# facebookresearch/hyperreel

Measured on NVIDIA H100. Metric: Mrays/s at 65k-ray x 32-sample batch, higher is better.
Workload: dtype f32 (sample net bf16x3 split on wgmma, fp32 accumulate)

## Files before the change

### hyperreel_b200/csrc/hr_api.cu

```cuda
#include <cuda_runtime.h>

#include <cmath>
#include <cstdarg>
#include <cstdio>
#include <cstring>
#include <limits>
#include <new>
#include <string>
#include <vector>

#include "hr_common.cuh"
#include "hr_encode.cuh"
#include "hr_geom.cuh"
#include "hr_mlp.cuh"
#include "hyperreel_b200.h"

namespace hr {
cudaError_t launch_render(const hr_config& cfg, const Derived& dv, const RenderTabs& tabs, const float* rays,
                          const float* heads, const RgbDst& rgb, long long n, const ExtraOut* so, int num_sms,
                          cudaStream_t stream, unsigned char* rgb8);
cudaError_t launch_render_bwd(const hr_config& cfg, const Derived& dv, const RenderTabs& tabs, const GradTabs& gt, const float* rays,
                              const float* heads, const float* d_rgb, float* d_heads, long long n, int clamp_output, int white_bg,
                              int num_sms, cudaStream_t stream);
cudaError_t launch_generate_rays(const hr_camera& cam, int c_in, long long first, long long n, float* out, cudaStream_t st);
// ... 6 lines not shown
static thread_local std::string g_err;

int hr_fail(const char* fmt, ...) {
  char buf[1024];
  va_list ap;
  va_start(ap, fmt);
  vsnprintf(buf, sizeof(buf), fmt, ap);
  va_end(ap);
  g_err = buf;
  return 1;
}

struct DeviceGuard {
  int prev = -1;
  bool switched = false;
  explicit DeviceGuard(int dev) {
    if (cudaGetDevice(&prev) == cudaSuccess && prev != dev) switched = (cudaSetDevice(dev) == cudaSuccess);
  }
  ~DeviceGuard() {
    if (switched) cudaSetDevice(prev);
  }
};

#define CK(expr)                                                                                                        \
  do {                                                                                                                  \
    cudaError_t _e = (expr);                                                                                            \
    if (_e != cudaSuccess) return hr_fail("%s failed: %s (%s:%d)", #expr, cudaGetErrorString(_e), __FILE__, __LINE__); \
  } while (0)

#include "hr_handle.h"

namespace {

__global__ void pack_channel_last(const float* __restrict__ src, float* __restrict__ dst, int C, int H, int W) {
  long long total = (long long)C * H * W;
  for (long long i = blockIdx.x * (long long)blockDim.x + threadIdx.x; i < total; i += (long long)gridDim.x * blockDim.x) {
    int c = (int)(i % C);
    long long hw = i / C;
    dst[i] = src[(long long)c * H * W + hw];
  }
}

__global__ void pack_time_lines(const float* __restrict__ src, float* __restrict__ dst, int C, int K, int L, float inv_fac,
                                float time_scale, float time_offset) {
  long long total = (long long)K * L * C;
  for (long long i = blockIdx.x * (long long)blockDim.x + threadIdx.x; i < total; i += (long long)gridDim.x * blockDim.x) {
    int c = (int)(i % C);
    int l = (int)((i / C) % L);
    int k = (int)(i / ((long long)C * L));
    float ft;
    int it = hr::keyframe_blend(k, K, inv_fac, time_scale, time_offset, ft);
    float a = src[((long long)c * K + it) * L + l];
    float b = src[((long long)c * K + it + 1) * L + l];
    dst[i] = __fmul_rn(1.0f - ft, a) + __fmul_rn(ft, b);
  }
}

__global__ void pack_simt_layer(const float* __restrict__ Wsrc, const float* __restrict__ bsrc, float* __restrict__ Wt,
                                float* __restrict__ bias, int Kp, int Np, int out_ch, int in_ch_src, int in_enc,
                                int in_pad, int has_input, int has_hidden, int width, int perm_S, int perm_stride) {
  long long total = (long long)Kp * Np;
  for (long long i = blockIdx.x * (long long)blockDim.x + threadIdx.x; i < total + Np; i += (long long)gridDim.x * blockDim.x) {
    if (i >= total) {
      int n = (int)(i - total);
      int ns = n;
      if (perm_S > 0 && n < out_ch) ns = (n % perm_S) * perm_stride + (n / perm_S);
      bias[n] = (n < out_ch) ? bsrc[ns] : 0.0f;
      continue;
    }
    int n = (int)(i % Np);
    int k = (int)(i / Np);
    float v = 0.0f;
    if (n < out_ch) {
      int ns = n;
      if (perm_S > 0) ns = (n % perm_S) * perm_stride + (n / perm_S);
      int ks = -1;
      if (has_input) {
        if (k < in_pad) ks = (k < in_enc) ? k : -1;
        else if (has_hidden) ks = in_enc + (k - in_pad);
      } else {
        ks = k;
      }
      if (ks >= 0 && ks < in_ch_src && (has_input || k < width)) v = Wsrc[(long long)ns * in_ch_src + ks];
    }
    Wt[i] = v;
  }
}
// ... 303 lines not shown
    float *Wt = nullptr, *bias = nullptr;
    if ((r = dev_alloc(h, (void**)&Wt, (size_t)Kp * Np * sizeof(float)))) break;
    if ((r = dev_alloc(h, (void**)&bias, (size_t)Np * sizeof(float)))) break;
    pack_simt_layer<<<grid_for((long long)Kp * Np + Np), 256, 0, st>>>(
        w_dev[l], b_dev[l], Wt, bias, Kp, Np, out_ch, in_src, nc.mlp_in, in_pad, (first || skip) ? 1 : 0, skip ? 1 : 0, W,
        last ? nc.n_samples : 0, nc.head_stride);
    simt.Wt[l] = Wt;
    simt.bias[l] = bias;
    simt.Kp[l] = Kp;
    simt.Np[l] = Np;
  }
  if (!r && nc.mlp_mode == HR_MLP_BF16X3_TC) {
    r = hr::pack_mlp_tc2(net, w_dev, b_dev, st);
    if (!r) net.tc_ready = true;
  }
  return r;
}

int hr_upload(hr_handle* h, const hr_params* p, void* stream) {
  if (!h || !p) return hr_fail("hr_upload: null argument");
  DeviceGuard guard(h->device);
  drop_host_graph(h);
  cudaStream_t st = (cudaStream_t)stream;
  const hr_config& c = h->cfg;
  h->slot_cursor = 0;
  h->uploaded = false;
  h->net.tc_ready = h->pre.tc_ready = false;
  std::vector<void*> temps;
  int rc = 0;

  rc = pack_net(h, h->net, p->mlp_weight, p->mlp_bias, p->on_device, st, temps);
  if (!rc && c.cascade) rc = pack_net(h, h->pre, p->pre_mlp_weight, p->pre_mlp_bias, p->on_device, st, temps);

  auto pack_tab = [&](const float* src, int C, int H, int Wd, const float** out) -> int {
    *out = nullptr;
    if (C == 0) return 0;
    if (!src) return hr_fail("hr_upload: table with C=%d missing", C);
    const float* d = nullptr;
    if (stage_in(src, (size_t)C * H * Wd, p->on_device, st, temps, &d)) return 1;
    float* dst = nullptr;
    if (dev_alloc(h, (void**)&dst, (size_t)C * H * Wd * sizeof(float))) return 1;
    pack_channel_last<<<grid_for((long long)C * H * Wd), 256, 0, st>>>(d, dst, C, H, Wd);
    *out = dst;
    return 0;
  };
  int n_app_total = 0;
  for (int i = 0; i < 3 && !rc; ++i) {
    const int C = c.n_sigma[i];
    n_app_total += c.n_app[i];
    const int H2 = c.dynamic ? c.num_keyframes : 1;
    hr::PlaneTab& ts = h->tabs.sig[i];
    hr::PlaneTab& ta = h->tabs.app[i];
    ts.C = C; ta.C = c.n_app[i];
    ts.H = ta.H = p->plane_h[i];
    ts.W = ta.W = p->plane_w[i];
    ts.H2 = ta.H2 = H2;
    ts.L = ta.L = p->second_len[i];
    if (C > 0 && (ts.H < 2 || ts.W < 2 || ts.L < 2)) { rc = hr_fail("hr_upload: plane %d too small (%dx%d, L=%d)", i, ts.H, ts.W, ts.L); break; }
    if ((rc = pack_tab(p->sigma_plane[i], C, ts.H, ts.W, &ts.space))) break;
    if ((rc = pack_tab(p->app_plane[i], C, ts.H, ts.W, &ta.space))) break;
    if (!c.dynamic) {
      if ((rc = pack_tab(p->sigma_second[i], C, H2, ts.L, &ts.second))) break;
      if ((rc = pack_tab(p->app_second[i], C, H2, ts.L, &ta.second))) break;
    } else if (C > 0) {
      if (H2 < 2) { rc = hr_fail("hr_upload: the keyframe (time) planes need at least 2 keyframes"); break; }
      for (int f = 0; f < 2 && !rc; ++f) {
        const float* srcp = f ? p->app_second[i] : p->sigma_second[i];
        if (!srcp) { rc = hr_fail("hr_upload: time plane %d missing", i); break; }
        const float* d = nullptr;
        if ((rc = stage_in(srcp, (size_t)C * H2 * ts.L, p->on_device, st, temps, &d))) break;
        float* dst = nullptr;
        if ((rc = dev_alloc(h, (void**)&dst, (size_t)C * H2 * ts.L * sizeof(float)))) break;
        pack_time_lines<<<grid_for((long long)C * H2 * ts.L), 256, 0, st>>>(d, dst, C, H2, ts.L, h->dv.time_inv_fac,
                                                                            h->dv.time_scale, h->dv.time_offset);
        (f ? ta.second : ts.second) = dst;
      }
      if (rc) break;
    }
  }
  if (!rc) {
    const int rx = p->plane_w[0], ry = p->plane_h[0], rz = p->second_len[0];
    h->dv.res[0] = rx; h->dv.res[1] = ry; h->dv.res[2] = rz;
    h->dv.kt = c.dynamic ? c.num_keyframes : 1;
    if (c.dynamic && c.num_keyframes < 2) rc = hr_fail("hr_upload: the keyframe (time) planes need at least 2 keyframes");
    if (c.n_sigma[1] > 0 && (p->plane_w[1] != rx || p->plane_h[1] != rz || p->second_len[1] != ry))
      rc = hr_fail("hr_upload: table group 1 is inconsistent with grid %dx%dx%d", rx, ry, rz);
    if (!rc && c.n_sigma[2] > 0 && (p->plane_w[2] != ry || p->plane_h[2] != rz || p->second_len[2] != rx))
      rc = hr_fail("hr_upload: table group 2 is inconsistent with grid %dx%dx%d", rx, ry, rz);
  }
  if (!rc) {
    if (!p->basis_mat) rc = hr_fail("hr_upload: basis_mat missing");
    else {
      const float* d = nullptr;
      size_t cnt = (size_t)c.app_dim * n_app_total;
      rc = stage_in(p->basis_mat, cnt, p->on_device, st, temps, &d);
      if (!rc) {
        float* dst = nullptr;
        rc = dev_alloc(h, (void**)&dst, cnt * sizeof(float));
        if (!rc) {
          cudaError_t e = cudaMemcpyAsync(dst, d, cnt * sizeof(float), cudaMemcpyDeviceToDevice, st);
          if (e != cudaSuccess) rc = hr_fail("basis copy failed: %s", cudaGetErrorString(e));
          h->tabs.basis = dst;
          h->tabs.n_app_total = n_app_total;
        }
      }
    }
  }
  if (!rc) {
    h->tabs.color_embedding = nullptr;
    if (c.n_color_views > 0) {
      if (!p->color_embedding) rc = hr_fail("hr_upload: color_embedding missing (n_color_views = %d)", c.n_color_views);
// ... 1053 lines not shown
```

### hyperreel_b200/csrc/hr_common.cuh

```cuda
#pragma once
#include <cuda_runtime.h>
#include <stdint.h>
#include "hyperreel_b200.h"

namespace hr {

struct PlaneTab {
  const float* space;
  const float* second;
  int H, W;
  int H2, L;
  int C;
};

struct RenderTabs {
  PlaneTab sig[3];
  PlaneTab app[3];
  const float* basis;
  int n_app_total;
  const float* color_embedding;
};

struct GradTabs {
  float* sig_space[3];
  float* sig_second[3];
  float* app_space[3];
  float* app_second[3];
  float* basis;
  float* color_embedding;
};

struct Derived {
  float time_fac;
  float time_inv_fac;
  float time_scale;
  float time_offset;
  float kf_max;
  float inv_end_dist;
  float dist_scale_fac;
  float inv_end_rad;
  float rad_scale_fac;
  int res[3];
  int kt;
};

struct RgbDst {
// ... 49 lines not shown
```

### hyperreel_b200/csrc/hr_render_bwd_kernel.cuh

```cuda
#pragma once
#include "hr_common.cuh"
#include "hr_geom.cuh"

namespace hr {

static constexpr int kBwdWarps = 4;

__device__ __forceinline__ float act_grad(const hr_act& a, float x) {
  const float v = __fadd_rn(__fmul_rn(x, a.inner_fac), a.shift);
  float g = 1.0f;
  if (a.kind == HR_ACT_SIGMOID) {
    const float s = 1.0f / (1.0f + expf(-v));
    g = s * (1.0f - s);
  } else if (a.kind == HR_ACT_TANH) {
    const float t = tanhf(v);
    g = 1.0f - t * t;
  }
  return g * a.inner_fac * a.outer_fac;
}

__device__ __forceinline__ float act_grad_eased(const hr_act& a, float x) {
  const float g = act_grad(a, x);
  return a.eased ? g * a.ease_mul : g;
}
// ... 81 lines not shown
    g[2] = (hz - hu * uz) / nn * cfg.plane_normal_scale;
    g[3] = cfg.z_scale * dpd_dpre / ddn;
  }
}

__device__ __forceinline__ void contract_point_vjp(const hr_config& cfg, const Derived& dv, float px, float py, float pz,
                                                   float& vx, float& vy, float& vz) {
  const float sr = cfg.contract_start_radius;
  const float x = px / sr, y = py / sr, z = pz / sr;
  const float r = sqrtf(x * x + y * y + z * z);
  if (r < 1.0f) {
    vx /= sr; vy /= sr; vz /= sr;
    return;
  }
  const float k0 = 2.0f + dv.inv_end_rad * dv.rad_scale_fac;
  const float g = k0 / r - dv.rad_scale_fac / (r * r);
  const float gp = -k0 / (r * r) + 2.0f * dv.rad_scale_fac / (r * r * r);
  const float xv = x * vx + y * vy + z * vz;
  const float s = gp / r * xv;
  vx = (g * vx + s * x) / sr;
  vy = (g * vy + s * y) / sr;
  vz = (g * vz + s * z) / sr;
}

__device__ __forceinline__ void red_add4(float* p, float a, float b, float c, float d) {
  asm volatile("red.global.add.v4.f32 [%0], {%1, %2, %3, %4};" ::"l"(p), "f"(a), "f"(b), "f"(c), "f"(d) : "memory");
}

struct Quad {
  float A[4], dAa[4], dAb[4];
  float B[4], dBc[4];
};

template <int C>
__device__ __forceinline__ void quad_fetch(Quad& q, const PlaneTab& T, int ia, int ib, int ic, int krow, int ch0, float fa, float fb,
                                           float fc) {
  const float* s0 = T.space + ((long long)(ib * T.W + ia) * C + ch0);
  const float4 v00 = ldg4(s0), v10 = ldg4(s0 + C), v01 = ldg4(s0 + (long long)T.W * C), v11 = ldg4(s0 + (long long)T.W * C + C);
  const float* e0 = T.second + ((long long)(krow * T.L + ic) * C + ch0);
  const float4 l0 = ldg4(e0), l1 = ldg4(e0 + C);
  const float a00[4] = {v00.x, v00.y, v00.z, v00.w}, a10[4] = {v10.x, v10.y, v10.z, v10.w};
  const float a01[4] = {v01.x, v01.y, v01.z, v01.w}, a11[4] = {v11.x, v11.y, v11.z, v11.w};
  const float b0[4] = {l0.x, l0.y, l0.z, l0.w}, b1[4] = {l1.x, l1.y, l1.z, l1.w};
#pragma unroll
  for (int c = 0; c < 4; ++c) {
    const float top = a00[c] + fa * (a10[c] - a00[c]);
    const float bot = a01[c] + fa * (a11[c] - a01[c]);
    q.A[c] = top + fb * (bot - top);
    q.dAa[c] = (1.0f - fb) * (a10[c] - a00[c]) + fb * (a11[c] - a01[c]);
    q.dAb[c] = bot - top;
    q.B[c] = b0[c] + fc * (b1[c] - b0[c]);
    q.dBc[c] = b1[c] - b0[c];
  }
}

template <int C>
__device__ __forceinline__ void quad_scatter(const Quad& q, const float (&g)[4], float* gspace, float* gsecond, const PlaneTab& T,
                                             int ia, int ib, int ic, int krow, int ch0, float fa, float fb, float fc, float& dfa,
                                             float& dfb, float& dfc) {
  float gA[4], gB[4];
#pragma unroll
  for (int c = 0; c < 4; ++c) {
    gA[c] = g[c] * q.B[c];
    gB[c] = g[c] * q.A[c];
    dfa += gA[c] * q.dAa[c];
    dfb += gA[c] * q.dAb[c];
    dfc += gB[c] * q.dBc[c];
  }
  float* s0 = gspace + ((long long)(ib * T.W + ia) * C + ch0);
  const float w00 = (1.0f - fa) * (1.0f - fb), w10 = fa * (1.0f - fb), w01 = (1.0f - fa) * fb, w11 = fa * fb;
  red_add4(s0, w00 * gA[0], w00 * gA[1], w00 * gA[2], w00 * gA[3]);
  red_add4(s0 + C, w10 * gA[0], w10 * gA[1], w10 * gA[2], w10 * gA[3]);
  red_add4(s0 + (long long)T.W * C, w01 * gA[0], w01 * gA[1], w01 * gA[2], w01 * gA[3]);
  red_add4(s0 + (long long)T.W * C + C, w11 * gA[0], w11 * gA[1], w11 * gA[2], w11 * gA[3]);
  float* e0 = gsecond + ((long long)(krow * T.L + ic) * C + ch0);
  const float u0 = 1.0f - fc, u1 = fc;
  red_add4(e0, u0 * gB[0], u0 * gB[1], u0 * gB[2], u0 * gB[3]);
  red_add4(e0 + C, u1 * gB[0], u1 * gB[1], u1 * gB[2], u1 * gB[3]);
}

struct BwdOpts {
  int clamp_output;
  int white_bg;
};

template <int SPL, bool DYN, int C0, int C1, int C2, int SHADE, bool RARE, bool EASE>
__global__ void __launch_bounds__(kBwdWarps * 32)
render_bwd_kernel(const __grid_constant__ hr_config cfg, const __grid_constant__ Derived dv,
                  const __grid_constant__ RenderTabs tabs, const __grid_constant__ GradTabs gt, const float* __restrict__ rays,
                  const float* __restrict__ heads, const float* __restrict__ d_rgb, float* __restrict__ d_heads,
                  long long n_rays, BwdOpts opt) {
  constexpr int NT = C0 + C1 + C2;
  constexpr int ROWS = (SHADE == HR_SHADE_SH) ? 9 : 1;
  constexpr int NB = 3 * ROWS * NT;
  extern __shared__ float smem[];
  float* s_basis = smem;
  float* s_gbasis = smem + NB;
  float* s_warp = smem + 2 * NB;
  constexpr int WARP_FLOATS = 3 * NT + 12 + 64;
  float* s_gemb = s_warp + kBwdWarps * WARP_FLOATS;
  const int n_emb = RARE ? 12 * cfg.n_color_views : 0;
  for (int i = threadIdx.x; i < NB; i += blockDim.x) { s_basis[i] = tabs.basis[i]; s_gbasis[i] = 0.0f; }
  if constexpr (RARE) {
    for (int i = threadIdx.x; i < n_emb; i += blockDim.x) s_gemb[i] = 0.0f;
  }
  __syncthreads();

  const int lane = threadIdx.x & 31, wib = threadIdx.x >> 5;
  float* Gs = s_warp + wib * WARP_FLOATS;
  float* Ys = Gs + 3 * NT;
  float* perm = Ys + 12;
  const int S = cfg.n_samples;
  const int out_stride = cfg.mlp_out;
  const long long warp0 = (long long)blockIdx.x * kBwdWarps + wib;
  const long long nwarps = (long long)gridDim.x * kBwdWarps;
  const float inv_x = __fdiv_rn(2.0f, __fsub_rn(cfg.aabb[3], cfg.aabb[0]));
  const float inv_y = __fdiv_rn(2.0f, __fsub_rn(cfg.aabb[4], cfg.aabb[1]));
  const float inv_z = __fdiv_rn(2.0f, __fsub_rn(cfg.aabb[5], cfg.aabb[2]));
  const float tsx = inv_x * 0.5f * (float)(dv.res[0] - 1), tsy = inv_y * 0.5f * (float)(dv.res[1] - 1),
              tsz = inv_z * 0.5f * (float)(dv.res[2] - 1);

  for (long long ray = warp0; ray < n_rays; ray += nwarps) {
    const float* r = rays + ray * cfg.c_in;
    const float* hrow = heads + ray * (long long)out_stride;
    float* grow = d_heads + ray * (long long)out_stride;
    const float ox = __ldg(r + 0), oy = __ldg(r + 1), oz = __ldg(r + 2);
    const float dx = __ldg(r + 3), dy = __ldg(r + 4), dz = __ldg(r + 5);
// ... 144 lines not shown
      dist[j] = t;
      const bool inside = !((cfg.aabb[0] > px) || (px > cfg.aabb[3]) || (cfg.aabb[1] > py) || (py > cfg.aabb[4]) ||
                            (cfg.aabb[2] > pz) || (pz > cfg.aabb[5]));
      valid[j] = act && inside && (t > 0.0f);
      const float ux = __fsub_rn(__fmul_rn(__fsub_rn(px, cfg.aabb[0]), inv_x), 1.0f);
      const float uy = __fsub_rn(__fmul_rn(__fsub_rn(py, cfg.aabb[1]), inv_y), 1.0f);
      const float uz = __fsub_rn(__fmul_rn(__fsub_rn(pz, cfg.aabb[2]), inv_z), 1.0f);
      const float tx = __fmul_rn(__fmul_rn(__fadd_rn(ux, 1.0f), 0.5f), (float)(dv.res[0] - 1));
      const float ty = __fmul_rn(__fmul_rn(__fadd_rn(uy, 1.0f), 0.5f), (float)(dv.res[1] - 1));
      const float tz = __fmul_rn(__fmul_rn(__fadd_rn(uz, 1.0f), 0.5f), (float)(dv.res[2] - 1));
      ix[j] = max(0, min((int)floorf(tx), dv.res[0] - 2));
      iy[j] = max(0, min((int)floorf(ty), dv.res[1] - 2));
      iz[j] = max(0, min((int)floorf(tz), dv.res[2] - 2));
      fx[j] = tx - (float)ix[j];
      fy[j] = ty - (float)iy[j];
      fz[j] = tz - (float)iz[j];
      if (!valid[j]) { ix[j] = 0; iy[j] = 0; iz[j] = 0; }
    }

    float feat[SPL], pre[SPL][3];
#pragma unroll
    for (int j = 0; j < SPL; ++j) {
      float sf = 0.0f, pr[3] = {0.0f, 0.0f, 0.0f};
      if (valid[j]) {
        int n0 = 0;
#pragma unroll
        for (int grp = 0; grp < 3; ++grp) {
          const int C = (grp == 0) ? C0 : ((grp == 1) ? C1 : C2);
          if (C == 0) continue;
          const int ia = (grp == 2) ? iy[j] : ix[j], ib = (grp == 0) ? iy[j] : iz[j], ic = (grp == 0) ? iz[j] : ((grp == 1) ? iy[j] : ix[j]);
          const float fa = (grp == 2) ? fy[j] : fx[j], fb = (grp == 0) ? fy[j] : fz[j], fc = (grp == 0) ? fz[j] : ((grp == 1) ? fy[j] : fx[j]);
          for (int ch0 = 0; ch0 < C; ch0 += 4) {
            Quad q;
            if (C == 8) quad_fetch<8>(q, tabs.sig[grp], ia, ib, ic, krow, ch0, fa, fb, fc);
            else quad_fetch<4>(q, tabs.sig[grp], ia, ib, ic, krow, ch0, fa, fb, fc);
#pragma unroll
            for (int c = 0; c < 4; ++c) sf = fmaf(q.A[c], q.B[c], sf);
            if (C == 8) quad_fetch<8>(q, tabs.app[grp], ia, ib, ic, krow, ch0, fa, fb, fc);
            else quad_fetch<4>(q, tabs.app[grp], ia, ib, ic, krow, ch0, fa, fb, fc);
#pragma unroll
            for (int c = 0; c < 4; ++c) {
              const float f = q.A[c] * q.B[c];
              const int n = n0 + ch0 + c;
              pr[0] = fmaf(Gs[n], f, pr[0]);
              pr[1] = fmaf(Gs[NT + n], f, pr[1]);
              pr[2] = fmaf(Gs[2 * NT + n], f, pr[2]);
            }
          }
          n0 += C;
        }
      }
      feat[j] = sf;
      pre[j][0] = pr[0]; pre[j][1] = pr[1]; pre[j][2] = pr[2];
    }

    float sigma[SPL], delta[SPL], ex[SPL], Tt[SPL], wgt[SPL], a1s[SPL];
    float cs[SPL][3], csh[SPL][3], rgbv[SPL][3];
    float carryT = 1.0f, accw = 0.0f, accC[3] = {0.f, 0.f, 0.f};
#pragma unroll
    for (int j = 0; j < SPL; ++j) {
      const int s = lane + 32 * j;
      const float* hp = hrow + ((s < S) ? s : 0);
      float sgm = feature2density(cfg, feat[j]);
      if (!valid[j]) sgm = 0.0f;
      sigma[j] = sgm;
      const SampleAlpha sa = sample_alpha<SPL>(dist, j, sigma[j], cfg.distance_scale, lane, S);
      delta[j] = sa.delta;
      ex[j] = sa.ex;
      a1s[j] = sa.a1;
      Tt[j] = transmittance<32>(sa.a1, lane, carryT);
      wgt[j] = sa.alpha * Tt[j];
      accw += wgt[j];
// ... 121 lines not shown
#pragma unroll
    for (int j = 0; j < SPL; ++j) {
      float prev = __shfl_up_sync(kFull, g_delta[j], 1);
      if (lane == 0) prev = (j > 0) ? __shfl_sync(kFull, g_delta[(j > 0) ? j - 1 : 0], 31) : 0.0f;
      else if (j > 0) (void)__shfl_sync(kFull, g_delta[j - 1], 31);
      g_dist[j] = prev - g_delta[j];
    }

    float g_head_cs[SPL][3], g_head_csh[SPL][3];
    float g_p[SPL][3];
#pragma unroll
    for (int j = 0; j < SPL; ++j) {
      const int s = lane + 32 * j;
      float gt3[3] = {0.0f, 0.0f, 0.0f};
      float g_feat = 0.0f;
      if (valid[j]) {
        if (cfg.fea2dense == HR_DENSE_RELU) g_feat = (feat[j] > 0.0f) ? g_sigma[j] : 0.0f;
        else if (cfg.fea2dense == HR_DENSE_RELU_ABS) g_feat = (feat[j] > 0.0f) ? g_sigma[j] : ((feat[j] < 0.0f) ? -g_sigma[j] : 0.0f);
        else { const float xs = feat[j] + cfg.density_shift; g_feat = g_sigma[j] / (1.0f + expf(-xs)); }
      }
      const bool any_app = (g_pre[j][0] != 0.0f) || (g_pre[j][1] != 0.0f) || (g_pre[j][2] != 0.0f);
      int n0 = 0;
#pragma unroll
      for (int grp = 0; grp < 3; ++grp) {
        const int C = (grp == 0) ? C0 : ((grp == 1) ? C1 : C2);
        if (C == 0) continue;
        const int ia = (grp == 2) ? iy[j] : ix[j], ib = (grp == 0) ? iy[j] : iz[j], ic = (grp == 0) ? iz[j] : ((grp == 1) ? iy[j] : ix[j]);
        const float fa = (grp == 2) ? fy[j] : fx[j], fb = (grp == 0) ? fy[j] : fz[j], fc = (grp == 0) ? fz[j] : ((grp == 1) ? fy[j] : fx[j]);
        float dfa = 0.0f, dfb = 0.0f, dfc = 0.0f;
        for (int ch0 = 0; ch0 < C; ch0 += 4) {
          Quad q;
          if (valid[j] && g_feat != 0.0f) {
            const float g4[4] = {g_feat, g_feat, g_feat, g_feat};
            if (C == 8) { quad_fetch<8>(q, tabs.sig[grp], ia, ib, ic, krow, ch0, fa, fb, fc); quad_scatter<8>(q, g4, gt.sig_space[grp], gt.sig_second[grp], tabs.sig[grp], ia, ib, ic, krow, ch0, fa, fb, fc, dfa, dfb, dfc); }
            else { quad_fetch<4>(q, tabs.sig[grp], ia, ib, ic, krow, ch0, fa, fb, fc); quad_scatter<4>(q, g4, gt.sig_space[grp], gt.sig_second[grp], tabs.sig[grp], ia, ib, ic, krow, ch0, fa, fb, fc, dfa, dfb, dfc); }
          }
          float m[3][4];
#pragma unroll
          for (int c = 0; c < 3; ++c)
#pragma unroll
            for (int k = 0; k < 4; ++k) m[c][k] = 0.0f;
          if (valid[j] && any_app) {
            if (C == 8) quad_fetch<8>(q, tabs.app[grp], ia, ib, ic, krow, ch0, fa, fb, fc);
            else quad_fetch<4>(q, tabs.app[grp], ia, ib, ic, krow, ch0, fa, fb, fc);
            float g4[4];
#pragma unroll
            for (int k = 0; k < 4; ++k) {
              const int n = n0 + ch0 + k;
              g4[k] = g_pre[j][0] * Gs[n] + g_pre[j][1] * Gs[NT + n] + g_pre[j][2] * Gs[2 * NT + n];
              const float f = q.A[k] * q.B[k];
              m[0][k] = g_pre[j][0] * f; m[1][k] = g_pre[j][1] * f; m[2][k] = g_pre[j][2] * f;
            }
            if (C == 8) quad_scatter<8>(q, g4, gt.app_space[grp], gt.app_second[grp], tabs.app[grp], ia, ib, ic, krow, ch0, fa, fb, fc, dfa, dfb, dfc);
            else quad_scatter<4>(q, g4, gt.app_space[grp], gt.app_second[grp], tabs.app[grp], ia, ib, ic, krow, ch0, fa, fb, fc, dfa, dfb, dfc);
          }
#pragma unroll
          for (int c = 0; c < 3; ++c)
#pragma unroll
            for (int k = 0; k < 4; ++k) {
              float v = m[c][k];
#pragma unroll
              for (int d = 1; d < 32; d <<= 1) v += __shfl_xor_sync(kFull, v, d);
              m[c][k] = v;
            }
          if constexpr (SHADE == HR_SHADE_SH) {
            for (int e = lane; e < 108; e += 32) {
              const int c = e / 36, rem = e % 36, kk = rem / 4, k = rem % 4;
              float v = (c == 0) ? m[0][0] : 0.0f;
#pragma unroll
              for (int cc = 0; cc < 3; ++cc)
#pragma unroll
                for (int k2 = 0; k2 < 4; ++k2)
                  if (cc == c && k2 == k) v = m[cc][k2];
              atomicAdd(&s_gbasis[(c * 9 + kk) * NT + n0 + ch0 + k], Ys[kk] * v);
            }
          } else {
            if (lane < 12) {
// ... 204 lines not shown
```

### hyperreel_b200/csrc/hr_render_kernel.cuh

```cuda
#pragma once
#include "hr_common.cuh"
#include "hr_geom.cuh"

namespace hr {

static constexpr int kWarpsPerCta = 8;
static constexpr int kMinCtasPerSm = 3;

template <int C, bool ROWS2>
struct Taps {
  float4 a, b;
};

template <int C, bool ROWS2>
__device__ __forceinline__ void fetch(Taps<C, ROWS2>& t, const float* __restrict__ tab, int off, int rs) {
  t.a = ldg4(tab + off);
  if constexpr (C == 8 && ROWS2) t.b = ldg4(tab + off + rs);
}

template <int C>
__device__ __forceinline__ void plane_share(const Taps<C, true>& t, float fa, float fb, int xt, int alt, float (&out)[4]) {
  const float wa = xt ? fa : 1.0f - fa;
  if constexpr (C == 8) {
    const float w0 = wa * (1.0f - fb), w1 = wa * fb;
    out[0] = fmaf(w1, t.b.x, w0 * t.a.x);
    out[1] = fmaf(w1, t.b.y, w0 * t.a.y);
    out[2] = fmaf(w1, t.b.z, w0 * t.a.z);
    out[3] = fmaf(w1, t.b.w, w0 * t.a.w);
  } else {
    const float w = wa * (alt ? fb : 1.0f - fb);
    out[0] = w * t.a.x; out[1] = w * t.a.y; out[2] = w * t.a.z; out[3] = w * t.a.w;
  }
}

template <int C>
__device__ __forceinline__ void line_full(const Taps<C, false>& t, float fc, int xt, float (&out)[4]) {
  const float wc = xt ? fc : 1.0f - fc;
  out[0] = wc * t.a.x; out[1] = wc * t.a.y; out[2] = wc * t.a.z; out[3] = wc * t.a.w;
#pragma unroll
  for (int c = 0; c < 4; ++c) out[c] += __shfl_xor_sync(kFull, out[c], 2);
}

template <int C, bool DYN>
struct GroupTaps {
  Taps<C, true> sp;
  Taps<C, false> se;
};

template <int C, bool DYN>
__device__ __forceinline__ void group_fetch(GroupTaps<C, DYN>& g, const PlaneTab& T, int ia, int ib, int ic, int krow, int xt,
                                            int alt, bool ok) {
  int so, eo;
  if constexpr (C == 8) {
    so = ((ib * T.W + ia + xt) << 3) + (alt << 2);
    eo = ((krow * T.L + ic + xt) << 3) + (alt << 2);
  } else {
    so = ((ib + alt) * T.W + ia + xt) << 2;
    eo = (krow * T.L + ic + xt) << 2;
  }
  so = ok ? so : 0;
  eo = ok ? eo : 0;
  fetch<C, true>(g.sp, T.space, so, T.W * C);
  fetch<C, false>(g.se, T.second, eo, 0);
}

template <int C, bool DYN>
__device__ __forceinline__ float group_sigma(const GroupTaps<C, DYN>& g, float fa, float fb, float fc, int xt, int alt) {
  float P[4], L[4];
  plane_share<C>(g.sp, fa, fb, xt, alt, P);
  line_full<C>(g.se, fc, xt, L);
  float s = (P[0] * L[0] + P[1] * L[1]) + (P[2] * L[2] + P[3] * L[3]);
  s += __shfl_xor_sync(kFull, s, 2);
  s += __shfl_xor_sync(kFull, s, 1);
  return s;
}

template <int C, bool DYN>
__device__ __forceinline__ void group_app(const GroupTaps<C, DYN>& g, float fa, float fb, float fc, int xt, int alt,
                                          float (&prod)[4]) {
  float P[4], L[4];
  plane_share<C>(g.sp, fa, fb, xt, alt, P);
  line_full<C>(g.se, fc, xt, L);
#pragma unroll
  for (int c = 0; c < 4; ++c) {
    P[c] += __shfl_xor_sync(kFull, P[c], 2);
    if constexpr (C == 4) P[c] += __shfl_xor_sync(kFull, P[c], 1);
    prod[c] = P[c] * L[c];
  }
}

template <int C, bool DYN>
__device__ __forceinline__ void group_accumulate(const GroupTaps<C, DYN>& sg, const GroupTaps<C, DYN>& ag, float fa, float fb,
                                                 float fc, int xt, int alt, const float* __restrict__ G0,
                                                 const float* __restrict__ G1, const float* __restrict__ G2, float (&v)[4]) {
  float P[4], L[4];
  plane_share<C>(sg.sp, fa, fb, xt, alt, P);
  line_full<C>(sg.se, fc, xt, L);
  v[3] += (P[0] * L[0] + P[1] * L[1]) + (P[2] * L[2] + P[3] * L[3]);
  plane_share<C>(ag.sp, fa, fb, xt, alt, P);
  line_full<C>(ag.se, fc, xt, L);
#pragma unroll
  for (int c = 0; c < 4; ++c) {
    const float t = P[c] * L[c];
    v[0] = fmaf(G0[c], t, v[0]);
    v[1] = fmaf(G1[c], t, v[1]);
    v[2] = fmaf(G2[c], t, v[2]);
  }
}

__device__ __forceinline__ float quad_transpose_reduce(const float (&v)[4], int xt, int alt) {
  const float x = __shfl_xor_sync(kFull, xt ? v[0] : v[2], 2);
  const float y = __shfl_xor_sync(kFull, xt ? v[1] : v[3], 2);
  const float k0 = (xt ? v[2] : v[0]) + x;
  const float k1 = (xt ? v[3] : v[1]) + y;
  const float z = __shfl_xor_sync(kFull, alt ? k0 : k1, 1);
  return (alt ? k1 : k0) + z;
}

template <int SPL, bool DYN, int C0, int C1, int C2, int SHADE, bool EXTRA, int RPW, bool RARE, bool EASE>
__global__ void __launch_bounds__(kWarpsPerCta * 32, SPL > 2 ? 1 : ((C1 + C2 == 0 || SPL == 1) ? 3 : 2))
render_kernel(const __grid_constant__ hr_config cfg, const __grid_constant__ Derived dv,
              const __grid_constant__ RenderTabs tabs, const float* __restrict__ rays,
              const float* __restrict__ heads, const __grid_constant__ RgbDst dst, long long n_rays, ExtraOut so,
              unsigned char* __restrict__ rgb8_out) {
  constexpr int NT = C0 + C1 + C2;
  constexpr int ROWS = (SHADE == HR_SHADE_SH) ? 9 : 1;
  constexpr int ROUNDS = 4 * SPL;
  constexpr int LW = 32 / RPW;
  static_assert(RPW == 1 || (SPL == 1 && !EXTRA), "two rays per warp: S <= 16, plain outputs");
  extern __shared__ float s_basis[];
  for (int i = threadIdx.x; i < 3 * ROWS * NT; i += blockDim.x) s_basis[i] = tabs.basis[i];
  __syncthreads();

  const int lane = threadIdx.x & 31;
  const int sub = lane / LW, sl = lane % LW;
  const int q = lane & 3, xt = q >> 1, alt = q & 1, quad = lane >> 2;
  const int qc = min(q, 2);
  const int S = cfg.n_samples;
  const int out_stride = cfg.mlp_out;
  const long long warp0 = (long long)blockIdx.x * kWarpsPerCta + (threadIdx.x >> 5);
  const long long nwarps = (long long)gridDim.x * kWarpsPerCta;

  constexpr int N0 = (C0 == 8) ? 4 : C0, N1 = (C1 == 8) ? 4 : C1, N2 = (C2 == 8) ? 4 : C2;
  constexpr int NTL = N0 + N1 + N2;
  int lcol[NTL];
#pragma unroll
  for (int i = 0; i < N0; ++i) lcol[i] = ((C0 == 8) ? alt * 4 : 0) + i;
#pragma unroll
  for (int i = 0; i < N1; ++i) lcol[N0 + i] = C0 + ((C1 == 8) ? alt * 4 : 0) + i;
#pragma unroll
  for (int i = 0; i < N2; ++i) lcol[N0 + N1 + i] = C0 + C1 + ((C2 == 8) ? alt * 4 : 0) + i;
  constexpr bool FOLD = (C1 + C2) > 0;
  constexpr int NG = (SHADE == HR_SHADE_SH) ? RPW : 1;
  float G[FOLD ? NG : 1][FOLD ? 3 : 1][FOLD ? NTL : 1];
  float Gr[FOLD ? 1 : NG][FOLD ? 1 : NT];
  int fcol[FOLD ? 1 : NT];
  if constexpr (!FOLD) {
#pragma unroll
    for (int i = 0; i < 4; ++i) { fcol[i] = alt * 4 + i; fcol[4 + i] = (1 - alt) * 4 + i; }
  }
// ... 197 lines not shown
        if (so.distances) so.distances[ray * S + s] = t;
        if (so.points) {
          so.points[(ray * S + s) * 3 + 0] = px;
          so.points[(ray * S + s) * 3 + 1] = py;
          so.points[(ray * S + s) * 3 + 2] = pz;
        }
      }
    }

    float sig_r[ROUNDS];
    float rgb_r[ROUNDS];
#pragma unroll
    for (int rd = 0; rd < ROUNDS; ++rd) {
      sig_r[rd] = 0.0f;
      rgb_r[rd] = 0.0f;
      if ((RPW == 1 ? rd : (rd % (LW / 8))) * 8 >= S) continue;
      const int j = rd >> 2;
      const int src = (rd & 3) * 8 + quad;
      const unsigned pxy = __shfl_sync(kFull, (unsigned)(ix[j] & 0xffff) | ((unsigned)iy[j] << 16), src);
      const unsigned pzk = __shfl_sync(kFull, (unsigned)iz[j] | ((unsigned)krow << 16), src);
      const int krow_s = (RPW == 1) ? krow : (int)(pzk >> 16);
      int sx = (int)(pxy & 0xffffu);
      if (sx == 0xffff) sx = -1;
      const int sy = (int)(pxy >> 16);
      const int sz = (int)(pzk & 0xffffu);
      const float gx = __shfl_sync(kFull, fx[j], src);
      const float gy = __shfl_sync(kFull, fy[j], src);
      const float gz = __shfl_sync(kFull, fz[j], src);
      const bool ok = sx >= 0;
      sx = max(sx, 0);
      GroupTaps<C0, DYN> s0, a0;
      GroupTaps<(C1 ? C1 : 4), DYN> s1, a1;
      GroupTaps<(C2 ? C2 : 4), DYN> s2, a2;
      group_fetch<C0, DYN>(s0, tabs.sig[0], sx, sy, sz, krow_s, xt, alt, ok);
      group_fetch<C0, DYN>(a0, tabs.app[0], sx, sy, sz, krow_s, xt, alt, ok);
      if constexpr (C1 > 0) {
        group_fetch<C1, DYN>(s1, tabs.sig[1], sx, sz, sy, krow_s, xt, alt, ok);
        group_fetch<C1, DYN>(a1, tabs.app[1], sx, sz, sy, krow_s, xt, alt, ok);
      }
      if constexpr (C2 > 0) {
        group_fetch<C2, DYN>(s2, tabs.sig[2], sy, sz, sx, krow_s, xt, alt, ok);
        group_fetch<C2, DYN>(a2, tabs.app[2], sy, sz, sx, krow_s, xt, alt, ok);
      }
      float col;
      if constexpr (FOLD) {
        float v4[4] = {0.0f, 0.0f, 0.0f, 0.0f};
        const int gr = (NG == 1) ? 0 : rd / (LW / 8);
        group_accumulate<C0, DYN>(s0, a0, gx, gy, gz, xt, alt, &G[gr][0][0], &G[gr][1][0], &G[gr][2][0], v4);
        if constexpr (C1 > 0)
          group_accumulate<C1, DYN>(s1, a1, gx, gz, gy, xt, alt, &G[gr][0][N0], &G[gr][1][N0], &G[gr][2][N0], v4);
        if constexpr (C2 > 0)
          group_accumulate<C2, DYN>(s2, a2, gy, gz, gx, xt, alt, &G[gr][0][N0 + N1], &G[gr][1][N0 + N1], &G[gr][2][N0 + N1], v4);
        const float acc = quad_transpose_reduce(v4, xt, alt);
        sig_r[rd] = ok ? acc : 0.0f;
        if constexpr (SHADE == HR_SHADE_SH) col = fmaxf(acc + 0.5f, 0.0f);
        else col = 1.0f / (1.0f + expf(-acc));
      } else {
        float f[NT];
        float sf = group_sigma<C0, DYN>(s0, gx, gy, gz, xt, alt);
        {
          float p[4];
          group_app<C0, DYN>(a0, gx, gy, gz, xt, alt, p);
#pragma unroll
          for (int c = 0; c < 4; ++c) f[c] = p[c];
          if constexpr (C0 == 8) {
#pragma unroll
            for (int c = 0; c < 4; ++c) f[4 + c] = __shfl_xor_sync(kFull, p[c], 1);
          }
        }
        if constexpr (C1 > 0) {
          float p[4];
          sf += group_sigma<C1, DYN>(s1, gx, gz, gy, xt, alt);
          group_app<C1, DYN>(a1, gx, gz, gy, xt, alt, p);
#pragma unroll
          for (int c = 0; c < 4; ++c) f[C0 + c] = p[c];
// ... 254 lines not shown
```

Before: 154.3.

## Interleave density and appearance tables per texel for co-located fetches

Packs each group's density and appearance planes and lines into one channel-last buffer with stride 2C, so both features of a texel sit side by side. The render and backward kernels take the table stride and feature offset as template parameters, so both fetches come from one base pointer and hit the same cache lines. This aims to improve cache-line and sector locality for the trilinear taps. It also adds a requirement that appearance and density channel counts match, and it leaves the gradient scatter paths on their old non-interleaved indexing.

```diff
diff --git a/hyperreel_b200/csrc/hr_api.cu b/hyperreel_b200/csrc/hr_api.cu
--- a/hyperreel_b200/csrc/hr_api.cu
+++ b/hyperreel_b200/csrc/hr_api.cu
@@ -62,27 +62,32 @@
 
 namespace {
 
-__global__ void pack_channel_last(const float* __restrict__ src, float* __restrict__ dst, int C, int H, int W) {
-  long long total = (long long)C * H * W;
+__global__ void pack_channel_last(const float* __restrict__ src0, const float* __restrict__ src1, float* dst0, float* dst1, int C,
+                                  int H, int W, int ts) {
+  long long total = 2LL * C * H * W;
   for (long long i = blockIdx.x * (long long)blockDim.x + threadIdx.x; i < total; i += (long long)gridDim.x * blockDim.x) {
-    int c = (int)(i % C);
-    long long hw = i / C;
-    dst[i] = src[(long long)c * H * W + hw];
-  }
-}
-
-__global__ void pack_time_lines(const float* __restrict__ src, float* __restrict__ dst, int C, int K, int L, float inv_fac,
-                                float time_scale, float time_offset) {
-  long long total = (long long)K * L * C;
+    const int c = (int)(i % C);
+    const int f = (int)((i / C) & 1);
+    const long long hw = i / (2 * C);
+    (f ? dst1 : dst0)[hw * ts + c] = (f ? src1 : src0)[(long long)c * H * W + hw];
+  }
+}
+
+__global__ void pack_time_lines(const float* __restrict__ src0, const float* __restrict__ src1, float* dst0, float* dst1, int C,
+                                int K, int L, int ts, float inv_fac, float time_scale, float time_offset) {
+  long long total = 2LL * K * L * C;
   for (long long i = blockIdx.x * (long long)blockDim.x + threadIdx.x; i < total; i += (long long)gridDim.x * blockDim.x) {
-    int c = (int)(i % C);
-    int l = (int)((i / C) % L);
-    int k = (int)(i / ((long long)C * L));
+    const int c = (int)(i % C);
+    const int f = (int)((i / C) & 1);
+    const long long kl = i / (2 * C);
+    const int l = (int)(kl % L);
+    const int k = (int)(kl / L);
+    const float* src = f ? src1 : src0;
     float ft;
     int it = hr::keyframe_blend(k, K, inv_fac, time_scale, time_offset, ft);
     float a = src[((long long)c * K + it) * L + l];
     float b = src[((long long)c * K + it + 1) * L + l];
-    dst[i] = __fmul_rn(1.0f - ft, a) + __fmul_rn(ft, b);
+    (f ? dst1 : dst0)[kl * ts + c] = __fmul_rn(1.0f - ft, a) + __fmul_rn(ft, b);
   }
 }
 
@@ -452,17 +457,15 @@
   rc = pack_net(h, h->net, p->mlp_weight, p->mlp_bias, p->on_device, st, temps);
   if (!rc && c.cascade) rc = pack_net(h, h->pre, p->pre_mlp_weight, p->pre_mlp_bias, p->on_device, st, temps);
 
-  auto pack_tab = [&](const float* src, int C, int H, int Wd, const float** out) -> int {
-    *out = nullptr;
-    if (C == 0) return 0;
-    if (!src) return hr_fail("hr_upload: table with C=%d missing", C);
-    const float* d = nullptr;
-    if (stage_in(src, (size_t)C * H * Wd, p->on_device, st, temps, &d)) return 1;
-    float* dst = nullptr;
-    if (dev_alloc(h, (void**)&dst, (size_t)C * H * Wd * sizeof(float))) return 1;
-    pack_channel_last<<<grid_for((long long)C * H * Wd), 256, 0, st>>>(d, dst, C, H, Wd);
-    *out = dst;
-    return 0;
+  const bool il = hr::tabs_interleaved(c.n_sigma[1], c.n_sigma[2]);
+  auto alloc_pair = [&](size_t n, int C, float** d0, float** d1) -> int {
+    if (il) {
+      if (dev_alloc(h, (void**)d0, 2 * n * sizeof(float))) return 1;
+      *d1 = *d0 + C;
+      return 0;
+    }
+    if (dev_alloc(h, (void**)d0, n * sizeof(float))) return 1;
+    return dev_alloc(h, (void**)d1, n * sizeof(float));
   };
   int n_app_total = 0;
   for (int i = 0; i < 3 && !rc; ++i) {
@@ -471,32 +474,41 @@
     const int H2 = c.dynamic ? c.num_keyframes : 1;
     hr::PlaneTab& ts = h->tabs.sig[i];
     hr::PlaneTab& ta = h->tabs.app[i];
-    ts.C = C; ta.C = c.n_app[i];
+    if (c.n_app[i] != C) { rc = hr_fail("hr_upload: group %d has %d appearance and %d density channels", i, c.n_app[i], C); break; }
+    ts.C = ta.C = C;
     ts.H = ta.H = p->plane_h[i];
     ts.W = ta.W = p->plane_w[i];
     ts.H2 = ta.H2 = H2;
     ts.L = ta.L = p->second_len[i];
-    if (C > 0 && (ts.H < 2 || ts.W < 2 || ts.L < 2)) { rc = hr_fail("hr_upload: plane %d too small (%dx%d, L=%d)", i, ts.H, ts.W, ts.L); break; }
-    if ((rc = pack_tab(p->sigma_plane[i], C, ts.H, ts.W, &ts.space))) break;
-    if ((rc = pack_tab(p->app_plane[i], C, ts.H, ts.W, &ta.space))) break;
-    if (!c.dynamic) {
-      if ((rc = pack_tab(p->sigma_second[i], C, H2, ts.L, &ts.second))) break;
-      if ((rc = pack_tab(p->app_second[i], C, H2, ts.L, &ta.second))) break;
-    } else if (C > 0) {
-      if (H2 < 2) { rc = hr_fail("hr_upload: the keyframe (time) planes need at least 2 keyframes"); break; }
-      for (int f = 0; f < 2 && !rc; ++f) {
-        const float* srcp = f ? p->app_second[i] : p->sigma_second[i];
-        if (!srcp) { rc = hr_fail("hr_upload: time plane %d missing", i); break; }
-        const float* d = nullptr;
-        if ((rc = stage_in(srcp, (size_t)C * H2 * ts.L, p->on_device, st, temps, &d))) break;
-        float* dst = nullptr;
-        if ((rc = dev_alloc(h, (void**)&dst, (size_t)C * H2 * ts.L * sizeof(float)))) break;
-        pack_time_lines<<<grid_for((long long)C * H2 * ts.L), 256, 0, st>>>(d, dst, C, H2, ts.L, h->dv.time_inv_fac,
-                                                                            h->dv.time_scale, h->dv.time_offset);
-        (f ? ta.second : ts.second) = dst;
-      }
-      if (rc) break;
-    }
+    ts.space = ta.space = ts.second = ta.second = nullptr;
+    if (C == 0) continue;
+    if (ts.H < 2 || ts.W < 2 || ts.L < 2) { rc = hr_fail("hr_upload: plane %d too small (%dx%d, L=%d)", i, ts.H, ts.W, ts.L); break; }
+    if (c.dynamic && H2 < 2) { rc = hr_fail("hr_upload: the keyframe (time) planes need at least 2 keyframes"); break; }
+    const int tstride = il ? 2 * C : C;
+    const size_t nsp = (size_t)C * ts.H * ts.W, nse = (size_t)C * H2 * ts.L;
+    const float *d0 = nullptr, *d1 = nullptr;
+    float *o0 = nullptr, *o1 = nullptr;
+    if (!p->sigma_plane[i] || !p->app_plane[i]) { rc = hr_fail("hr_upload: table with C=%d missing", C); break; }
+    if ((rc = stage_in(p->sigma_plane[i], nsp, p->on_device, st, temps, &d0))) break;
+    if ((rc = stage_in(p->app_plane[i], nsp, p->on_device, st, temps, &d1))) break;
+    if ((rc = alloc_pair(nsp, C, &o0, &o1))) break;
+    pack_channel_last<<<grid_for(2LL * nsp), 256, 0, st>>>(d0, d1, o0, o1, C, ts.H, ts.W, tstride);
+    ts.space = o0;
+    ta.space = o1;
+    if (!p->sigma_second[i] || !p->app_second[i]) {
+      rc = c.dynamic ? hr_fail("hr_upload: time plane %d missing", i) : hr_fail("hr_upload: table with C=%d missing", C);
+      break;
+    }
+    if ((rc = stage_in(p->sigma_second[i], nse, p->on_device, st, temps, &d0))) break;
+    if ((rc = stage_in(p->app_second[i], nse, p->on_device, st, temps, &d1))) break;
+    if ((rc = alloc_pair(nse, C, &o0, &o1))) break;
+    if (c.dynamic)
+      pack_time_lines<<<grid_for(2LL * nse), 256, 0, st>>>(d0, d1, o0, o1, C, H2, ts.L, tstride, h->dv.time_inv_fac,
+                                                           h->dv.time_scale, h->dv.time_offset);
+    else
+      pack_channel_last<<<grid_for(2LL * nse), 256, 0, st>>>(d0, d1, o0, o1, C, H2, ts.L, tstride);
+    ts.second = o0;
+    ta.second = o1;
   }
   if (!rc) {
     const int rx = p->plane_w[0], ry = p->plane_h[0], rz = p->second_len[0];
diff --git a/hyperreel_b200/csrc/hr_common.cuh b/hyperreel_b200/csrc/hr_common.cuh
--- a/hyperreel_b200/csrc/hr_common.cuh
+++ b/hyperreel_b200/csrc/hr_common.cuh
@@ -12,6 +12,8 @@
   int H2, L;
   int C;
 };
+
+__host__ __device__ constexpr bool tabs_interleaved(int c1, int c2) { return c1 + c2 > 0; }
 
 struct RenderTabs {
   PlaneTab sig[3];
diff --git a/hyperreel_b200/csrc/hr_render_bwd_kernel.cuh b/hyperreel_b200/csrc/hr_render_bwd_kernel.cuh
--- a/hyperreel_b200/csrc/hr_render_bwd_kernel.cuh
+++ b/hyperreel_b200/csrc/hr_render_bwd_kernel.cuh
@@ -137,13 +137,13 @@
   float B[4], dBc[4];
 };
 
-template <int C>
+template <int C, int TS>
 __device__ __forceinline__ void quad_fetch(Quad& q, const PlaneTab& T, int ia, int ib, int ic, int krow, int ch0, float fa, float fb,
                                            float fc) {
-  const float* s0 = T.space + ((long long)(ib * T.W + ia) * C + ch0);
-  const float4 v00 = ldg4(s0), v10 = ldg4(s0 + C), v01 = ldg4(s0 + (long long)T.W * C), v11 = ldg4(s0 + (long long)T.W * C + C);
-  const float* e0 = T.second + ((long long)(krow * T.L + ic) * C + ch0);
-  const float4 l0 = ldg4(e0), l1 = ldg4(e0 + C);
+  const float* s0 = T.space + ((long long)(ib * T.W + ia) * TS + ch0);
+  const float4 v00 = ldg4(s0), v10 = ldg4(s0 + TS), v01 = ldg4(s0 + (long long)T.W * TS), v11 = ldg4(s0 + (long long)T.W * TS + TS);
+  const float* e0 = T.second + ((long long)(krow * T.L + ic) * TS + ch0);
+  const float4 l0 = ldg4(e0), l1 = ldg4(e0 + TS);
   const float a00[4] = {v00.x, v00.y, v00.z, v00.w}, a10[4] = {v10.x, v10.y, v10.z, v10.w};
   const float a01[4] = {v01.x, v01.y, v01.z, v01.w}, a11[4] = {v11.x, v11.y, v11.z, v11.w};
   const float b0[4] = {l0.x, l0.y, l0.z, l0.w}, b1[4] = {l1.x, l1.y, l1.z, l1.w};
@@ -198,6 +198,7 @@
   constexpr int NT = C0 + C1 + C2;
   constexpr int ROWS = (SHADE == HR_SHADE_SH) ? 9 : 1;
   constexpr int NB = 3 * ROWS * NT;
+  constexpr int IL = tabs_interleaved(C1, C2) ? 2 : 1;
   extern __shared__ float smem[];
   float* s_basis = smem;
   float* s_gbasis = smem + NB;
@@ -408,12 +409,12 @@
           const float fa = (grp == 2) ? fy[j] : fx[j], fb = (grp == 0) ? fy[j] : fz[j], fc = (grp == 0) ? fz[j] : ((grp == 1) ? fy[j] : fx[j]);
           for (int ch0 = 0; ch0 < C; ch0 += 4) {
             Quad q;
-            if (C == 8) quad_fetch<8>(q, tabs.sig[grp], ia, ib, ic, krow, ch0, fa, fb, fc);
-            else quad_fetch<4>(q, tabs.sig[grp], ia, ib, ic, krow, ch0, fa, fb, fc);
+            if (C == 8) quad_fetch<8, IL * 8>(q, tabs.sig[grp], ia, ib, ic, krow, ch0, fa, fb, fc);
+            else quad_fetch<4, IL * 4>(q, tabs.sig[grp], ia, ib, ic, krow, ch0, fa, fb, fc);
 #pragma unroll
             for (int c = 0; c < 4; ++c) sf = fmaf(q.A[c], q.B[c], sf);
-            if (C == 8) quad_fetch<8>(q, tabs.app[grp], ia, ib, ic, krow, ch0, fa, fb, fc);
-            else quad_fetch<4>(q, tabs.app[grp], ia, ib, ic, krow, ch0, fa, fb, fc);
+            if (C == 8) quad_fetch<8, IL * 8>(q, tabs.app[grp], ia, ib, ic, krow, ch0, fa, fb, fc);
+            else quad_fetch<4, IL * 4>(q, tabs.app[grp], ia, ib, ic, krow, ch0, fa, fb, fc);
 #pragma unroll
             for (int c = 0; c < 4; ++c) {
               const float f = q.A[c] * q.B[c];
@@ -601,8 +602,8 @@
           Quad q;
           if (valid[j] && g_feat != 0.0f) {
             const float g4[4] = {g_feat, g_feat, g_feat, g_feat};
-            if (C == 8) { quad_fetch<8>(q, tabs.sig[grp], ia, ib, ic, krow, ch0, fa, fb, fc); quad_scatter<8>(q, g4, gt.sig_space[grp], gt.sig_second[grp], tabs.sig[grp], ia, ib, ic, krow, ch0, fa, fb, fc, dfa, dfb, dfc); }
-            else { quad_fetch<4>(q, tabs.sig[grp], ia, ib, ic, krow, ch0, fa, fb, fc); quad_scatter<4>(q, g4, gt.sig_space[grp], gt.sig_second[grp], tabs.sig[grp], ia, ib, ic, krow, ch0, fa, fb, fc, dfa, dfb, dfc); }
+            if (C == 8) { quad_fetch<8, IL * 8>(q, tabs.sig[grp], ia, ib, ic, krow, ch0, fa, fb, fc); quad_scatter<8>(q, g4, gt.sig_space[grp], gt.sig_second[grp], tabs.sig[grp], ia, ib, ic, krow, ch0, fa, fb, fc, dfa, dfb, dfc); }
+            else { quad_fetch<4, IL * 4>(q, tabs.sig[grp], ia, ib, ic, krow, ch0, fa, fb, fc); quad_scatter<4>(q, g4, gt.sig_space[grp], gt.sig_second[grp], tabs.sig[grp], ia, ib, ic, krow, ch0, fa, fb, fc, dfa, dfb, dfc); }
           }
           float m[3][4];
 #pragma unroll
@@ -610,8 +611,8 @@
 #pragma unroll
             for (int k = 0; k < 4; ++k) m[c][k] = 0.0f;
           if (valid[j] && any_app) {
-            if (C == 8) quad_fetch<8>(q, tabs.app[grp], ia, ib, ic, krow, ch0, fa, fb, fc);
-            else quad_fetch<4>(q, tabs.app[grp], ia, ib, ic, krow, ch0, fa, fb, fc);
+            if (C == 8) quad_fetch<8, IL * 8>(q, tabs.app[grp], ia, ib, ic, krow, ch0, fa, fb, fc);
+            else quad_fetch<4, IL * 4>(q, tabs.app[grp], ia, ib, ic, krow, ch0, fa, fb, fc);
             float g4[4];
 #pragma unroll
             for (int k = 0; k < 4; ++k) {
diff --git a/hyperreel_b200/csrc/hr_render_kernel.cuh b/hyperreel_b200/csrc/hr_render_kernel.cuh
--- a/hyperreel_b200/csrc/hr_render_kernel.cuh
+++ b/hyperreel_b200/csrc/hr_render_kernel.cuh
@@ -47,20 +47,20 @@
   Taps<C, false> se;
 };
 
-template <int C, bool DYN>
+template <int C, bool DYN, int TS, int FO>
 __device__ __forceinline__ void group_fetch(GroupTaps<C, DYN>& g, const PlaneTab& T, int ia, int ib, int ic, int krow, int xt,
                                             int alt, bool ok) {
   int so, eo;
   if constexpr (C == 8) {
-    so = ((ib * T.W + ia + xt) << 3) + (alt << 2);
-    eo = ((krow * T.L + ic + xt) << 3) + (alt << 2);
+    so = (ib * T.W + ia + xt) * TS + (alt << 2) + FO;
+    eo = (krow * T.L + ic + xt) * TS + (alt << 2) + FO;
   } else {
-    so = ((ib + alt) * T.W + ia + xt) << 2;
-    eo = (krow * T.L + ic + xt) << 2;
+    so = ((ib + alt) * T.W + ia + xt) * TS + FO;
+    eo = (krow * T.L + ic + xt) * TS + FO;
   }
   so = ok ? so : 0;
   eo = ok ? eo : 0;
-  fetch<C, true>(g.sp, T.space, so, T.W * C);
+  fetch<C, true>(g.sp, T.space, so, T.W * TS);
   fetch<C, false>(g.se, T.second, eo, 0);
 }
 
@@ -126,6 +126,7 @@
   constexpr int NT = C0 + C1 + C2;
   constexpr int ROWS = (SHADE == HR_SHADE_SH) ? 9 : 1;
   constexpr int ROUNDS = 4 * SPL;
+  constexpr int IL = tabs_interleaved(C1, C2) ? 2 : 1;
   constexpr int LW = 32 / RPW;
   static_assert(RPW == 1 || (SPL == 1 && !EXTRA), "two rays per warp: S <= 16, plain outputs");
   extern __shared__ float s_basis[];
@@ -389,15 +390,15 @@
       GroupTaps<C0, DYN> s0, a0;
       GroupTaps<(C1 ? C1 : 4), DYN> s1, a1;
       GroupTaps<(C2 ? C2 : 4), DYN> s2, a2;
-      group_fetch<C0, DYN>(s0, tabs.sig[0], sx, sy, sz, krow_s, xt, alt, ok);
-      group_fetch<C0, DYN>(a0, tabs.app[0], sx, sy, sz, krow_s, xt, alt, ok);
+      group_fetch<C0, DYN, IL * C0, 0>(s0, tabs.sig[0], sx, sy, sz, krow_s, xt, alt, ok);
+      group_fetch<C0, DYN, IL * C0, (IL - 1) * C0>(a0, (IL == 2 ? tabs.sig : tabs.app)[0], sx, sy, sz, krow_s, xt, alt, ok);
       if constexpr (C1 > 0) {
-        group_fetch<C1, DYN>(s1, tabs.sig[1], sx, sz, sy, krow_s, xt, alt, ok);
-        group_fetch<C1, DYN>(a1, tabs.app[1], sx, sz, sy, krow_s, xt, alt, ok);
+        group_fetch<C1, DYN, IL * C1, 0>(s1, tabs.sig[1], sx, sz, sy, krow_s, xt, alt, ok);
+        group_fetch<C1, DYN, IL * C1, (IL - 1) * C1>(a1, (IL == 2 ? tabs.sig : tabs.app)[1], sx, sz, sy, krow_s, xt, alt, ok);
       }
       if constexpr (C2 > 0) {
-        group_fetch<C2, DYN>(s2, tabs.sig[2], sy, sz, sx, krow_s, xt, alt, ok);
-        group_fetch<C2, DYN>(a2, tabs.app[2], sy, sz, sx, krow_s, xt, alt, ok);
+        group_fetch<C2, DYN, IL * C2, 0>(s2, tabs.sig[2], sy, sz, sx, krow_s, xt, alt, ok);
+        group_fetch<C2, DYN, IL * C2, (IL - 1) * C2>(a2, (IL == 2 ? tabs.sig : tabs.app)[2], sy, sz, sx, krow_s, xt, alt, ok);
       }
       float col;
       if constexpr (FOLD) {
```

Result: no change. 154.5 (median of 6 runs) (+0.1%).
